# GuillaumeHolley/BloomFilterTrie

Hardware: AMD Instinct MI355X
Metric: M k-mers/sec queried (presenceNode) (higher is better)
Workload: dtype u64

## Files before the change

### bloomfiltertrie_amd/csrc/bft_kh.hip

```cpp
#include <hip/hip_runtime.h>

#include <algorithm>
#include <atomic>
#include <cstring>

#include "bft_dev.h"
#include "bft_image.h"
#include "bft_kh.h"
#include "bft_claims.h"
#include "bft_walk.h"
#include "bft_kernels_load.h"
#include "bft_kernels_seqwin.h"
#include "bft_kh_dev.h"
#include "bft_scan.h"
#include "bft_rows16.h"
#include "bft_sort.h"

#define BFT_KH_MIN_CLAIM 4u
#define BFT_KH_MAX_CLAIM 64u
typedef BftClaims<BFT_KH_MIN_CLAIM> KhClaims;
template <int W, int S>
__global__ __launch_bounds__(BFT_KH_BLOCK) void k_query_kh(BftImage im, const uint8_t* __restrict__ packed, uint64_t n, int B, uint64_t* __restrict__ bits64,
                                                          uint32_t* __restrict__ out32, BftClaimCtr ctr, uint32_t chunk) {
    const uint64_t end_aligned = ((uint64_t)packed + n * (uint64_t)B) & ~3ull;
    const uint64_t nblk = (n + BFT_KH_BLOCK - 1) / BFT_KH_BLOCK, nwords = (n + 63) / 64;
    constexpr uint32_t WPB = BFT_KH_BLOCK / 64;
    __shared__ uint32_t s_next[2];
    __shared__ uint64_t s_bits[BFT_KH_MAX_CLAIM * WPB];
    __shared__ uint4 s_lines[WPB][64 * BFT_KH_LDS_LINE];
    uint4* const wave_lines = s_lines[threadIdx.x >> 6];
    const uint4* const mine = wave_lines + (threadIdx.x & 63u) * BFT_KH_LDS_LINE;
    KhClaims cl(ctr, chunk, nblk, s_next);
    cl.first();
    while (cl.blk < nblk) {
        const uint64_t i = cl.blk * BFT_KH_BLOCK + threadIdx.x;
        const bool live = i < n;
        BftKhKey<W> key;
        key.home = 0;
        key.field = 0;
#pragma unroll
        for (int w = 0; w < W; w++) { key.body[w] = 0; key.bmask[w] = 0; }
        uint64_t t[W];
#pragma unroll
        for (int w = 0; w < W; w++) t[w] = 0;
        if (live) {
            uint64_t x[W];
            load_x<W>(packed, i, B, end_aligned, x);
            bft_tform_from_x<W>(x, im.k, t);
            bft_kh_key<W>(t, im.k, im.kh, key);
        }
        kh_fetch_quad(im, key.home, live, wave_lines);
        bool present = false;
        uint32_t val = 0xFFFFFFFFu;
        if (live) {
            int res = kh_lds_scan<W, S>(im, mine, key, 0u, &val);
            for (uint32_t d = 1; res < 0 && d <= im.kh.maxd; d++) {
                const uint64_t* line = im.kh_lines + (key.home + d) * BFT_KH_LINE_WORDS;
                uint64_t hd[2];
                bft_kh_load_header(line, hd);
                res = bft_kh_scan<W, S>(im, line, hd, key, d, &val);
            }
            if (res < 0 && im.kh_ovf_n) res = bft_kh_overflow_find<W>(im, t, &val) ? 1 : 0;
            present = res > 0;
        }
        const uint64_t mask = __ballot(present);
        if (out32 && i < n) out32[i] = present ? val : 0xFFFFFFFFu;
        if ((threadIdx.x & 63u) == 0) s_bits[(cl.blk - cl.start) * WPB + (threadIdx.x >> 6)] = mask;
        if (cl.last_of_round()) {
            __syncthreads();
            const uint64_t w0 = cl.start * WPB, w1 = min(nwords, cl.blk_end * WPB);
            if (w0 + threadIdx.x < w1) __builtin_nontemporal_store(s_bits[threadIdx.x], &bits64[w0 + threadIdx.x]);
        }
        cl.advance();
    }
    cl.done();
}

template <int W, int S>
__global__ __launch_bounds__(256) void k_color_rows_kh(BftImage im, const uint8_t* __restrict__ packed, uint64_t n, int B, uint64_t* __restrict__ bits64,
                                                       const uint8_t* __restrict__ bm, uint32_t stride, uint32_t rowbytes, uint32_t tile_rows, uint32_t div_m, uint32_t div_l,
                                                       uint8_t* __restrict__ out) {
    __shared__ uint4 s_lines[4][64 * BFT_KH_LDS_LINE];
    __shared__ uint32_t s_cs_all[4][BFT_KH_ROWS_TILE + 1];
    const uint64_t end_aligned = ((uint64_t)packed + n * (uint64_t)B) & ~3ull;
    const uint64_t ntiles = (n + tile_rows - 1) / tile_rows;
    const uint32_t lane = threadIdx.x & 63u, wave = threadIdx.x >> 6;
    uint4* const wave_lines = s_lines[wave];
    const uint4* const mine = wave_lines + lane * BFT_KH_LDS_LINE;
    uint32_t* const s_cs = s_cs_all[wave];
    for (uint64_t tile = (uint64_t)blockIdx.x * 4u + wave; tile < ntiles; tile += (uint64_t)gridDim.x * 4u) {
        const uint64_t q0 = tile * tile_rows;
        const uint32_t nt = (uint32_t)min((uint64_t)tile_rows, n - q0);
        __builtin_amdgcn_wave_barrier();
#pragma unroll 1
        for (uint32_t j0 = 0; j0 < nt; j0 += 64u) {
            const uint64_t i = q0 + j0 + lane;
            const bool live = i < n;
            BftKhKey<W> key;
            key.home = 0;
            key.field = 0;
#pragma unroll
            for (int w = 0; w < W; w++) { key.body[w] = 0; key.bmask[w] = 0; }
            uint64_t t[W];
#pragma unroll
            for (int w = 0; w < W; w++) t[w] = 0;
            if (live) {
                uint64_t x[W];
                load_x<W>(packed, i, B, end_aligned, x);
                bft_tform_from_x<W>(x, im.k, t);
                bft_kh_key<W>(t, im.k, im.kh, key);
            }
            kh_fetch_quad(im, key.home, live, wave_lines);
            bool present = false;
            uint32_t val = 0;
            if (live) {
                int res = kh_lds_scan<W, S>(im, mine, key, 0u, &val);
                for (uint32_t d = 1; res < 0 && d <= im.kh.maxd; d++) {
                    const uint64_t* line = im.kh_lines + (key.home + d) * BFT_KH_LINE_WORDS;
                    uint64_t hd[2];
                    bft_kh_load_header(line, hd);
                    res = bft_kh_scan<W, S>(im, line, hd, key, d, &val);
                }
                if (res < 0 && im.kh_ovf_n) res = bft_kh_overflow_find<W>(im, t, &val) ? 1 : 0;
                present = res > 0;
            }
            s_cs[j0 + lane] = present ? val * (stride >> 2) : CR16_ABSENT;
            const uint64_t mask = __ballot(present);
            if (lane == 0) bits64[(q0 + j0) >> 6] = mask;
        }
        if (lane == 0) s_cs[nt] = CR16_ABSENT;
        __builtin_amdgcn_fence(__ATOMIC_RELEASE, "wavefront");
        __builtin_amdgcn_wave_barrier();
        __builtin_amdgcn_fence(__ATOMIC_ACQUIRE, "wavefront");
        cr16_stream_tile(s_cs, nt, rowbytes, div_m, div_l, bm, out + q0 * rowbytes, lane);
    }
}

#ifndef BFT_KH_CT
#define BFT_KH_CT 4
#endif
#ifndef BFT_KH_LEN_T
#define BFT_KH_LEN_T uint16_t
#endif
template <int W, int S>
__global__ __launch_bounds__(BFT_KH_BLOCK) void k_colors_kh(BftImage im, const uint8_t* __restrict__ packed, uint64_t n, int B, uint64_t* __restrict__ bits64,
                                                           unsigned long long* __restrict__ offsets, uint32_t* __restrict__ ids, uint64_t ids_cap, unsigned long long* __restrict__ needed,
                                                           unsigned long long* __restrict__ scratch) {
    constexpr uint32_t WPB = BFT_KH_BLOCK / 64, CT = BFT_KH_CT;
    constexpr unsigned long long F_AGG = 1ull << 62, F_INC = 2ull << 62, VMASK = (1ull << 62) - 1ull;
    __shared__ uint4 s_lines[WPB][64 * BFT_KH_LDS_LINE];
    __shared__ uint64_t s_bits[CT * WPB];
    __shared__ uint32_t s_sum[CT * WPB];
    __shared__ BFT_KH_LEN_T s_len[CT * BFT_KH_BLOCK];
    __shared__ uint32_t s_src[CT * BFT_KH_BLOCK];
    __shared__ uint32_t s_tile;
    __shared__ unsigned long long s_prefix;
    const uint64_t end_aligned = ((uint64_t)packed + n * (uint64_t)B) & ~3ull;
    const uint32_t lane = threadIdx.x & 63u, wave = threadIdx.x >> 6;
    uint4* const wave_lines = s_lines[wave];
    const uint4* const mine = wave_lines + lane * BFT_KH_LDS_LINE;
    const uint64_t ntiles = (n + (uint64_t)CT * BFT_KH_BLOCK - 1) / ((uint64_t)CT * BFT_KH_BLOCK), nwords = (n + 63) / 64;
    unsigned long long* states = scratch + 1;
    for (;;) {
        if (threadIdx.x == 0) s_tile = (uint32_t)atomicAdd(scratch, 1ull);
        __syncthreads();
        const uint64_t tile = s_tile;
        if (tile >= ntiles) return;
#pragma unroll 1
        for (uint32_t c = 0; c < CT; c++) {
            const uint64_t i = (tile * CT + c) * BFT_KH_BLOCK + threadIdx.x;
            const bool live = i < n;
            BftKhKey<W> key;
            key.home = 0;
            key.field = 0;
#pragma unroll
            for (int w = 0; w < W; w++) { key.body[w] = 0; key.bmask[w] = 0; }
            uint64_t t[W];
#pragma unroll
            for (int w = 0; w < W; w++) t[w] = 0;
            if (live) {
                uint64_t x[W];
                load_x<W>(packed, i, B, end_aligned, x);
                bft_tform_from_x<W>(x, im.k, t);
                bft_kh_key<W>(t, im.k, im.kh, key);
            }
            kh_fetch_quad(im, key.home, live, wave_lines);
            bool present = false;
            uint32_t val = 0;
            if (live) {
                int res = kh_lds_scan<W, S>(im, mine, key, 0u, &val);
                for (uint32_t d = 1; res < 0 && d <= im.kh.maxd; d++) {
                    const uint64_t* line = im.kh_lines + (key.home + d) * BFT_KH_LINE_WORDS;
                    uint64_t hd[2];
                    bft_kh_load_header(line, hd);
                    res = bft_kh_scan<W, S>(im, line, hd, key, d, &val);
                }
                if (res < 0 && im.kh_ovf_n) res = bft_kh_overflow_find<W>(im, t, &val) ? 1 : 0;
                present = res > 0;
            }
            s_src[c * BFT_KH_BLOCK + threadIdx.x] = present ? val : 0xFFFFFFFFu;
            const uint64_t mask = __ballot(present);
            if (lane == 0) s_bits[c * WPB + wave] = mask;
        }
        {
            uint32_t cs[CT], o0[CT], o1[CT];
#pragma unroll
            for (uint32_t c = 0; c < CT; c++) cs[c] = s_src[c * BFT_KH_BLOCK + threadIdx.x];
#pragma unroll
            for (uint32_t c = 0; c < CT; c++) {
                o0[c] = 0; o1[c] = 0;
                if (cs[c] != 0xFFFFFFFFu) { o0[c] = im.cs_off[cs[c]]; o1[c] = im.cs_off[cs[c] + 1]; }
            }
#pragma unroll
            for (uint32_t c = 0; c < CT; c++) {
                const uint32_t len = o1[c] - o0[c];
                s_len[c * BFT_KH_BLOCK + threadIdx.x] = (BFT_KH_LEN_T)len;
                s_src[c * BFT_KH_BLOCK + threadIdx.x] = o0[c];
                uint32_t ws = len;
#pragma unroll
                for (int o = 32; o > 0; o >>= 1) ws += __shfl_down(ws, o);
                if (lane == 0) s_sum[c * WPB + wave] = ws;
            }
        }
        __syncthreads();
        {
            const uint64_t w0 = tile * CT * WPB;
            if (threadIdx.x < CT * WPB && w0 + threadIdx.x < nwords) __builtin_nontemporal_store(s_bits[threadIdx.x], &bits64[w0 + threadIdx.x]);
        }
        if (wave == 0) {
            unsigned long long total = lane < CT * WPB ? s_sum[lane] : 0u;
#pragma unroll
            for (int o = 32; o > 0; o >>= 1) total += __shfl_down(total, o);
            total = __shfl(total, 0);
            unsigned long long ex = 0;
            if (tile == 0) {
                if (lane == 0) __hip_atomic_store(&states[0], F_INC | (total & VMASK), __ATOMIC_RELAXED, __HIP_MEMORY_SCOPE_AGENT);
            } else {
                if (lane == 0) __hip_atomic_store(&states[tile], F_AGG | (total & VMASK), __ATOMIC_RELAXED, __HIP_MEMORY_SCOPE_AGENT);
                long long first = (long long)tile - 1;
                for (;;) {
                    const long long tt = first - (long long)lane;
                    unsigned long long st = F_INC;
                    if (tt >= 0) {
                        do { st = __hip_atomic_load(&states[tt], __ATOMIC_RELAXED, __HIP_MEMORY_SCOPE_AGENT); } while ((st >> 62) == 0ull && (__builtin_amdgcn_s_sleep(1), true));
                    }
                    const uint64_t incl = __ballot((st >> 62) == 2ull);
                    const int stop = incl ? __builtin_ctzll(incl) : 64;
                    unsigned long long x = ((int)lane <= stop && tt >= 0) ? (st & VMASK) : 0ull;
#pragma unroll
                    for (int o = 32; o > 0; o >>= 1) x += __shfl_down(x, o);
                    ex += __shfl(x, 0);
                    if (stop < 64) break;
                    first -= 64;
                }
                if (lane == 0) __hip_atomic_store(&states[tile], F_INC | ((ex + total) & VMASK), __ATOMIC_RELAXED, __HIP_MEMORY_SCOPE_AGENT);
            }
            if (lane == 0) {
                s_prefix = ex;
                if (tile == ntiles - 1) {
                    offsets[n] = ex + total;
                    if (needed) *needed = ex + total;
                }
            }
        }
        __syncthreads();
        unsigned long long run = s_prefix;
#pragma unroll 1
        for (uint32_t c = 0; c < CT; c++) {
            const uint32_t len = s_len[c * BFT_KH_BLOCK + threadIdx.x], src = s_src[c * BFT_KH_BLOCK + threadIdx.x];
            unsigned long long wbase = run;
#pragma unroll
            for (uint32_t w = 0; w < WPB; w++) {
                if (w < wave) wbase += s_sum[c * WPB + w];
                run += s_sum[c * WPB + w];
            }
            uint32_t inc = len;
#pragma unroll
            for (int o = 1; o < 64; o <<= 1) {
                const uint32_t y = __shfl_up(inc, o);
                if ((int)lane >= o) inc += y;
            }
            const uint32_t ar = inc - len, span = __shfl(inc, 63);
            const uint64_t i = (tile * CT + c) * BFT_KH_BLOCK + threadIdx.x;
            if (i < n) offsets[i] = wbase + ar;
            if (!ids) continue;
            for (uint32_t r0 = 0; r0 < span; r0 += 64) {
                const uint32_t r = r0 + lane;
                const bool in = r < span;
                const uint32_t rr = in ? r : span - 1;
                uint32_t lo = 0, hi = 63;
#pragma unroll
                for (int it = 0; it < 6; it++) {
                    const uint32_t mid = (lo + hi + 1) >> 1;
                    const uint32_t am = __shfl(ar, mid);
                    if (am <= rr) lo = mid; else hi = mid - 1;
                }
                const uint32_t as = __shfl(ar, lo);
                const uint32_t ss = __shfl(src, lo);
                if (in && wbase + r < ids_cap) ids[wbase + r] = bft_cs_id_at(im.cs_ids, im.cs_w, ss + (r - as));
            }
        }
        __syncthreads();
    }
}

template <int W, int S>
__device__ __forceinline__ int kh_count4(const BftImage& im, const uint64_t* t0, uint32_t b, int wild_word, int wild_shift, bool live, uint4* wave_lines) {
    BftKhKey<W> key;
    key.home = 0; key.field = 0;
#pragma unroll
    for (int w = 0; w < W; w++) { key.body[w] = 0; key.bmask[w] = 0; }
    if (live) bft_kh_key<W>(t0, im.k, im.kh, key);
    kh_fetch_quad(im, key.home, live, wave_lines);
    if (!live) return 0;
    BftKhFamily<W> fam;
    bft_kh_family<W>(im.kh, key, b, fam);
    int count = 0;
    int res = kh_lds_count<W, S>(im, wave_lines + (threadIdx.x & 63u) * BFT_KH_LDS_LINE, key, fam, 0u, &count);
    for (uint32_t d = 1; res < 0 && count < 4 && d <= im.kh.maxd; d++) res = bft_kh_count_line<W, S>(im, im.kh_lines + (key.home + d) * BFT_KH_LINE_WORDS, key, fam, d, &count);
    if (res < 0 && count < 4 && im.kh_ovf_n) {
        for (int v = 0; v < 4; v++) {
            uint64_t c[W];
            uint32_t val;
#pragma unroll
            for (int w = 0; w < W; w++) c[w] = t0[w] | (w == wild_word ? (uint64_t)v << wild_shift : 0ull);
            count += bft_kh_overflow_find<W>(im, c, &val) ? 1 : 0;
        }
    }
    return count;
}

#define BFT_KH_BR_MAX_CLAIM 16u
template <int W, int S>
__global__ __launch_bounds__(BFT_KH_BLOCK) void k_branching_kh(BftImage im, const uint8_t* __restrict__ packed, uint64_t n, int B, uint64_t* __restrict__ bits64,
                                                              uint8_t* __restrict__ counts, BftClaimCtr ctr, uint32_t chunk) {
    const uint64_t end_aligned = ((uint64_t)packed + n * (uint64_t)B) & ~3ull;
    const uint64_t nblk = (n + BFT_KH_BLOCK - 1) / BFT_KH_BLOCK, nwords = (n + 63) / 64;
    constexpr uint32_t WPB = BFT_KH_BLOCK / 64;
    const int k = im.k, L = im.L, rb = 2 * (k - 9 * L);
    __shared__ uint32_t s_next[2];
    __shared__ uint64_t s_bits[BFT_KH_BR_MAX_CLAIM * WPB];
    __shared__ uint4 s_lines[WPB][64 * BFT_KH_LDS_LINE];
    uint4* const wave_lines = s_lines[threadIdx.x >> 6];
    KhClaims cl(ctr, chunk, nblk, s_next);
    cl.first();
    while (cl.blk < nblk) {
        const uint64_t i = cl.blk * BFT_KH_BLOCK + threadIdx.x;
        const bool live = i < n;
        uint64_t x[W], y[W], t[W];
#pragma unroll
        for (int w = 0; w < W; w++) x[w] = 0;
        if (live) load_x<W>(packed, i, B, end_aligned, x);
#pragma unroll
        for (int w = 0; w < W; w++) y[w] = (x[w] >> 2) | (w + 1 < W ? x[w + 1] << 62 : 0ull);
        bft_tform_from_x<W>(y, k, t);
        const int vo = rb ? 0 : 2;
        const int cr = kh_count4<W, S>(im, t, (uint32_t)vo, W - 1, vo, live, wave_lines);
        int cl_ = 0;
        const bool left = live && (counts || cr < 2);
        if (__any(left)) {
#pragma unroll
            for (int w = W - 1; w >= 0; w--) y[w] = (x[w] << 2) | (w > 0 ? x[w - 1] >> 62 : 0ull);
            const int top = 2 * k - 64 * (W - 1);
            if (top < 64) y[W - 1] &= (1ull << top) - 1ull;
            bft_tform_from_x<W>(y, k, t);
            const int o = rb + 18 * (L - 1), ow = W - 1 - (o >> 6), osh = o & 63;
            cl_ = kh_count4<W, S>(im, t, im.kh.po < 32u ? im.kh.restb - 2u : (uint32_t)o, ow, osh, left, wave_lines);
        }
        const int branching = live && (cr > 1 || cl_ > 1);
        if (counts && live) counts[i] = (uint8_t)((cr << 4) | cl_);
        const uint64_t mask = __ballot(branching);
        if ((threadIdx.x & 63u) == 0) s_bits[(cl.blk - cl.start) * WPB + (threadIdx.x >> 6)] = mask;
        if (cl.last_of_round()) {
            __syncthreads();
            const uint64_t w0 = cl.start * WPB, w1 = min(nwords, cl.blk_end * WPB);
            if (w0 + threadIdx.x < w1) __builtin_nontemporal_store(s_bits[threadIdx.x], &bits64[w0 + threadIdx.x]);
        }
        cl.advance();
    }
    cl.done();
}

template <int W, int S>
__global__ __launch_bounds__(256) void k_seq_kh(BftImage im, const uint64_t* __restrict__ codes, const uint32_t* __restrict__ bad, const uint64_t* __restrict__ seq_off,
                                                const uint64_t* __restrict__ pos_off, const uint32_t* __restrict__ tile_seq, uint32_t n_seqs, int canonical,
                                                uint32_t* __restrict__ csout, BftClaimCtr ctr, uint32_t chunk) {
    const uint64_t P = pos_off[n_seqs];
    const uint64_t nblk = (P + 255) / 256;
    __shared__ uint32_t s_next[2];
    __shared__ uint4 s_lines[4][64 * BFT_KH_LDS_LINE];
    uint4* const wave_lines = s_lines[threadIdx.x >> 6];
    KhClaims cl(ctr, chunk, nblk, s_next);
    cl.first();
    for (; cl.blk < nblk; cl.advance()) {
        const uint64_t p = cl.blk * 256 + threadIdx.x;
        uint32_t cs = 0xFFFFFFFFu;
        uint64_t x[W], t[W];
        BftKhKey<W> key;
        key.home = 0; key.field = 0;
#pragma unroll
        for (int w = 0; w < W; w++) { key.body[w] = 0; key.bmask[w] = 0; }
        bool live = false;
        if (p < P) {
            uint32_t lo = tile_seq[p >> 6];
            while (lo + 1 < n_seqs && pos_off[lo + 1] <= p) lo++;
            if (seq_window<W>(codes, bad, seq_off[lo] + (p - pos_off[lo]), im.k, canonical, x)) {
                bft_tform_from_x<W>(x, im.k, t);
                bft_kh_key<W>(t, im.k, im.kh, key);
                live = true;
            }
        }
        kh_fetch_quad(im, key.home, live, wave_lines);
        if (live) {
            uint32_t val = 0;
            int res = kh_lds_scan<W, S>(im, wave_lines + (threadIdx.x & 63u) * BFT_KH_LDS_LINE, key, 0u, &val);
            for (uint32_t d = 1; res < 0 && d <= im.kh.maxd; d++) {
                const uint64_t* line = im.kh_lines + (key.home + d) * BFT_KH_LINE_WORDS;
                uint64_t hd[2];
                bft_kh_load_header(line, hd);
                res = bft_kh_scan<W, S>(im, line, hd, key, d, &val);
            }
            if (res < 0 && im.kh_ovf_n) res = bft_kh_overflow_find<W>(im, t, &val) ? 1 : 0;
            if (res > 0) cs = val;
        }
        if (p < P) csout[p] = cs;
    }
    cl.done();
}

template <int W>
struct __attribute__((packed, aligned(4))) KhRec {
    uint64_t t[W];
    uint32_t v;
};
template <int W>
struct KhSortIn {
    const uint64_t* tk;
    const uint32_t* vals;
    int k;
    BftKhGeo g;
    __device__ __forceinline__ uint32_t key(uint32_t i) const {
        uint64_t t[W];
        BftKhKey<W> kk;
        bft_load_row<W>(tk + (uint64_t)i * W, t);
        bft_kh_key<W>(t, k, g, kk);
        return (uint32_t)kk.home;
    }
    __device__ __forceinline__ KhRec<W> val(uint32_t i) const {
        KhRec<W> r;
        bft_load_row<W>(tk + (uint64_t)i * W, r.t);
        r.v = vals[i];
        return r;
    }
};
#define BFT_KH_SCAN_BIAS (1ull << 40)
struct KhScanIn {
    const uint32_t* key_s;
    uint32_t S;
    __device__ __forceinline__ uint64_t operator()(uint64_t s) const { return BFT_KH_SCAN_BIAS + (uint64_t)key_s[s] * S - s; }
};
template <int W>
__global__ __launch_bounds__(256) void k_kh_assemble(const uint32_t* __restrict__ key_s, const KhRec<W>* __restrict__ rec_s, const uint64_t* __restrict__ vscan, uint64_t n, int k,
                                                     BftKhGeo g, uint32_t* __restrict__ status, uint64_t* __restrict__ kh, uint64_t* __restrict__ ovf_k,
                                                     uint32_t* __restrict__ ovf_v) {
    __shared__ unsigned long long s_line[4][64][BFT_KH_LINE_WORDS];
    uint32_t dmax = 0;
    const uint64_t n_lines = g.nl + BFT_KH_TAIL_LINES;
    const uint32_t wave = threadIdx.x >> 6, lane = threadIdx.x & 63u;
    const uint64_t nblk = (n + 255) / 256;
    for (uint64_t blk = blockIdx.x; blk < nblk; blk += gridDim.x) {
        const uint64_t s = blk * 256 + threadIdx.x;
        const bool live = s < n;
        uint64_t p = 0, ln = ~0ull;
        bool first_of_line = false, last_of_line = false;
        if (live) {
            p = vscan[s] - BFT_KH_SCAN_BIAS + s;
            ln = p / g.S;
            first_of_line = s == 0 || (vscan[s - 1] - BFT_KH_SCAN_BIAS + (s - 1)) / g.S != ln;
            last_of_line = s + 1 == n || (vscan[s + 1] - BFT_KH_SCAN_BIAS + (s + 1)) / g.S != ln;
        }
        const uint64_t heads = __ballot(live && (first_of_line || lane == 0));
        const uint32_t rank = (uint32_t)__popcll(heads & ((2ull << lane) - 1ull)) - 1u;
        const uint64_t firsts = __ballot(live && first_of_line), lasts = __ballot(live && last_of_line);
        const uint64_t my_head_bit = live ? (1ull << (63 - __builtin_clzll((heads & ((2ull << lane) - 1ull)) | 1ull))) : 0ull;
        const uint64_t above = heads & ~((my_head_bit << 1) - 1ull);
        const uint32_t my_last_lane = above ? (uint32_t)__builtin_ctzll(above) - 1u : 63u;
        const bool whole = live && (firsts & my_head_bit) && my_last_lane < 64u && ((lasts >> my_last_lane) & 1ull);
#pragma unroll
        for (uint32_t q = 0; q < BFT_KH_LINE_WORDS; q++) s_line[wave][lane][q] = 0ull;
        __builtin_amdgcn_wave_barrier();
        uint64_t img[BFT_KH_LINE_WORDS];
#pragma unroll
        for (uint32_t q = 0; q < BFT_KH_LINE_WORDS; q++) img[q] = 0;
        if (live) {
            const uint64_t home = key_s[s], d = ln - home;
            const KhRec<W> r = rec_s[s];
            if (ln >= n_lines) atomicOr(&status[0], 1u);
            else if (d > g.maxd) {
                const uint32_t at = atomicAdd(&status[3], 1u);
                if (at >= BFT_KH_OVF_CAP) atomicOr(&status[0], 1u);
                else {
#pragma unroll
                    for (int w = 0; w < W; w++) ovf_k[(size_t)at * W + w] = r.t[w];
                    ovf_v[at] = r.v;
                }
                img[1] = 1ull << (64u - g.S + (uint32_t)(p % g.S));
            } else {
                dmax = max(dmax, (uint32_t)d);
                bft_kh_slot_image<W>(r.t, k, g, (uint32_t)(p % g.S), (uint32_t)d, r.v, img);
            }
            if (ln < n_lines) {
                if (whole) {
#pragma unroll
                    for (uint32_t q = 0; q < BFT_KH_LINE_WORDS; q++)
                        if (img[q]) atomicOr(&s_line[wave][rank][q], (unsigned long long)img[q]);
                } else {
                    unsigned long long* line = (unsigned long long*)(kh + ln * BFT_KH_LINE_WORDS);
#pragma unroll
                    for (uint32_t q = 0; q < BFT_KH_LINE_WORDS; q++)
                        if (img[q]) atomicOr(&line[q], (unsigned long long)img[q]);
                }
            }
        }
        __builtin_amdgcn_wave_barrier();
        if (whole && first_of_line && ln < n_lines) {
            ulonglong2* dst = reinterpret_cast<ulonglong2*>(kh + ln * BFT_KH_LINE_WORDS);
#pragma unroll
            for (int q = 0; q < 4; q++) dst[q] = make_ulonglong2(s_line[wave][rank][2 * q], s_line[wave][rank][2 * q + 1]);
        }
        __builtin_amdgcn_wave_barrier();
    }
    for (int o = 32; o > 0; o >>= 1) dmax = max(dmax, (uint32_t)__shfl_down(dmax, o));
    if ((threadIdx.x & 63u) == 0 && dmax) atomicMax(&status[2], dmax);
}

template <int W>
static int kh_sort_w(const uint64_t* d_tk, const uint32_t* d_vals, uint64_t n, int k, const BftKhGeo& g, BftKhScratch& sc, hipStream_t s) {
    DevBuf &key = sc.b[0], &rec = sc.b[1], &key_s = sc.b[2], &rec_s = sc.b[3], &tmp = sc.b[6];
    unsigned bits = 1;
    while (bits < 32 && (g.nl >> bits)) bits++;
    CK(key_s.alloc(n * 4));
    CK(rec_s.alloc(n * sizeof(KhRec<W>)));
    if (bft_rs::make_plan(0u, bits).P > 1) {
        CK(key.alloc(n * 4));
        CK(rec.alloc(n * sizeof(KhRec<W>)));
    }
    CK((bft_rs::sort<uint32_t, KhRec<W>, KhSortIn<W>, bft_rs::SHAPE_BACK>(KhSortIn<W>{d_tk, d_vals, k, g}, n, key_s.as<uint32_t>(), rec_s.as<KhRec<W>>(), key.as<uint32_t>(), rec.as<KhRec<W>>(), 0u, bits, s, tmp)));
    HIPCK(hipGetLastError());
    return 0;
}
template <int W>
static int kh_lay_w(uint64_t n, int k, const BftKhGeo& g, uint64_t* d_kh, uint64_t* d_ovf_k, uint32_t* d_ovf_v, uint32_t* d_status, BftKhScratch& sc,
                    hipStream_t s) {
    DevBuf &key_s = sc.b[2], &rec_s = sc.b[3], &vs = sc.b[5], &tmp = sc.b[6];
    CK(vs.alloc(n * 8));
    const dim3 b(256);
    HIPCK(hipMemsetAsync(d_status, 0, 16, s));
    HIPCK(hipMemsetAsync(d_kh, 0, (g.nl + BFT_KH_TAIL_LINES) * BFT_KH_LINE_WORDS * 8, s));
    CK((bft_scan::scan<uint64_t, KhScanIn, bft_scan::Max, true>(KhScanIn{key_s.as<uint32_t>(), g.S}, vs.as<uint64_t>(), n, 0ull, bft_scan::Max(), s, tmp)));
    hipLaunchKernelGGL(k_kh_assemble<W>, dim3((unsigned)std::min<uint64_t>((n + 255) / 256, 256ull * 32)), b, 0, s, key_s.as<uint32_t>(), rec_s.as<KhRec<W>>(), vs.as<uint64_t>(), n, k, g,
                       d_status, d_kh, d_ovf_k, d_ovf_v);
    HIPCK(hipGetLastError());
    return 0;
}

template <int W>
static int kh_test_sort_w(int shape, const uint32_t* keys, const void* recs, uint64_t n, unsigned b0, unsigned b1, uint32_t* ok, void* orec, hipStream_t s, uint32_t* h_dbase) {
    typedef bft_rs::PtrIn<uint32_t, KhRec<W>> In;
    const In in{keys, (const KhRec<W>*)recs};
    if (shape == bft_rs::SHAPE_BACK) return bft_rs::sort_test_run<uint32_t, KhRec<W>, In, bft_rs::SHAPE_BACK>(in, n, ok, (KhRec<W>*)orec, b0, b1, s, h_dbase);
    if (shape == bft_rs::SHAPE_BIG) return bft_rs::sort_test_run<uint32_t, KhRec<W>, In, bft_rs::SHAPE_BIG>(in, n, ok, (KhRec<W>*)orec, b0, b1, s, h_dbase);
    return bft_fail(BFT_GPU_E_ARG, "test sort: shape");
}
int bft_kh_test_sort(int W, int shape, const uint32_t* keys, const void* recs, uint64_t n, unsigned b0, unsigned b1, uint32_t* ok, void* orec, hipStream_t s, uint32_t* h_dbase) {
    switch (W) {
    case 1: return kh_test_sort_w<1>(shape, keys, recs, n, b0, b1, ok, orec, s, h_dbase);
    case 2: return kh_test_sort_w<2>(shape, keys, recs, n, b0, b1, ok, orec, s, h_dbase);
    case 3: return kh_test_sort_w<3>(shape, keys, recs, n, b0, b1, ok, orec, s, h_dbase);
    case 4: return kh_test_sort_w<4>(shape, keys, recs, n, b0, b1, ok, orec, s, h_dbase);
    default: return bft_fail(BFT_GPU_E_ARG, "test sort: W");
    }
}
template <int W>
static uint32_t kh_test_tile_w(int shape) {
    return shape == bft_rs::SHAPE_BACK ? bft_rs::tile_entries<uint32_t, KhRec<W>, bft_rs::SHAPE_BACK>()
         : shape == bft_rs::SHAPE_BIG  ? bft_rs::tile_entries<uint32_t, KhRec<W>, bft_rs::SHAPE_BIG>() : 0u;
}
uint32_t bft_kh_test_sort_tile(int W, int shape) {
    return W == 1 ? kh_test_tile_w<1>(shape) : W == 2 ? kh_test_tile_w<2>(shape) : W == 3 ? kh_test_tile_w<3>(shape) : W == 4 ? kh_test_tile_w<4>(shape) : 0u;
}

int bft_kh_sort(const uint64_t* d_tk, const uint32_t* d_vals, uint64_t n, int k, int W, const BftKhGeo& g, BftKhScratch& sc, hipStream_t s) {
    switch (W) {
    case 1: return kh_sort_w<1>(d_tk, d_vals, n, k, g, sc, s);
    case 2: return kh_sort_w<2>(d_tk, d_vals, n, k, g, sc, s);
    case 3: return kh_sort_w<3>(d_tk, d_vals, n, k, g, sc, s);
    default: return kh_sort_w<4>(d_tk, d_vals, n, k, g, sc, s);
    }
}
int bft_kh_lay(uint64_t n, int k, int W, const BftKhGeo& g, uint64_t* d_kh, uint64_t* d_ovf_k, uint32_t* d_ovf_v, uint32_t* d_status, BftKhScratch& sc, hipStream_t s) {
    switch (W) {
    case 1: return kh_lay_w<1>(n, k, g, d_kh, d_ovf_k, d_ovf_v, d_status, sc, s);
    case 2: return kh_lay_w<2>(n, k, g, d_kh, d_ovf_k, d_ovf_v, d_status, sc, s);
    case 3: return kh_lay_w<3>(n, k, g, d_kh, d_ovf_k, d_ovf_v, d_status, sc, s);
    default: return kh_lay_w<4>(n, k, g, d_kh, d_ovf_k, d_ovf_v, d_status, sc, s);
    }
}

template <int W>
__global__ __launch_bounds__(256) void k_kh_dump(BftImage im, uint64_t* __restrict__ keys, uint64_t stride, uint32_t* __restrict__ vals, unsigned long long* __restrict__ cnt) {
    __shared__ uint32_t s_cnt;
    __shared__ unsigned long long s_base;
    const uint64_t n_lines = im.kh.nl + BFT_KH_TAIL_LINES;
    const uint32_t S = im.kh.S;
    for (uint64_t l0 = (uint64_t)blockIdx.x * blockDim.x; l0 < n_lines; l0 += (uint64_t)gridDim.x * blockDim.x) {
        const uint64_t ln = l0 + threadIdx.x;
        if (threadIdx.x == 0) s_cnt = 0;
        __syncthreads();
        uint64_t hd[2] = {0, 0};
        uint32_t occ = 0;
        const uint64_t* line = im.kh_lines + ln * BFT_KH_LINE_WORDS;
        if (ln < n_lines) {
            bft_kh_load_header(line, hd);
            occ = (uint32_t)(hd[1] >> (64u - S));
        }
        {
            uint32_t real = 0;
            const uint64_t vmask = (1ull << im.kh.cb) - 1ull;
            for (uint32_t o2 = occ; o2;) {
                const uint32_t s = (uint32_t)__builtin_ctz(o2);
                o2 &= o2 - 1u;
                uint64_t body[W];
                bft_kh_load_body<W>(line, s, im.kh.wb, body);
                if (body[0] & vmask) real |= 1u << s;
            }
            occ = real;
        }
        const uint32_t mine = (uint32_t)__popc(occ);
        uint32_t my_off = mine ? atomicAdd(&s_cnt, mine) : 0u;
        __syncthreads();
        if (threadIdx.x == 0) s_base = s_cnt ? atomicAdd(cnt, (unsigned long long)s_cnt) : 0ull;
        __syncthreads();
        uint64_t j = s_base + my_off;
        while (occ) {
            const uint32_t s = (uint32_t)__builtin_ctz(occ);
            occ &= occ - 1u;
            uint64_t t[W];
            uint32_t v;
            bft_kh_slot_decode<W>(im, line, hd, ln, s, t, &v);
#pragma unroll
            for (int i = 0; i < W; i++) keys[(uint64_t)i * stride + j] = t[i];
            vals[j] = v;
            j++;
        }
        __syncthreads();
    }
    if (blockIdx.x == 0) {
        __syncthreads();
        if (threadIdx.x == 0) s_base = im.kh_ovf_n ? atomicAdd(cnt, (unsigned long long)im.kh_ovf_n) : 0ull;
        __syncthreads();
        for (uint32_t e = threadIdx.x; e < im.kh_ovf_n; e += blockDim.x) {
#pragma unroll
            for (int i = 0; i < W; i++) keys[(uint64_t)i * stride + s_base + e] = im.kh_ovf[(size_t)e * W + i];
            vals[s_base + e] = im.kh_ovf_val[e];
        }
    }
}

int bft_kh_dump(const BftImage& im, uint64_t* d_keys, uint64_t stride, uint32_t* d_vals, unsigned long long* d_cnt, hipStream_t s) {
    const dim3 grid(256 * 8), block(256);
    switch (im.W) {
    case 1: hipLaunchKernelGGL(k_kh_dump<1>, grid, block, 0, s, im, d_keys, stride, d_vals, d_cnt); break;
    case 2: hipLaunchKernelGGL(k_kh_dump<2>, grid, block, 0, s, im, d_keys, stride, d_vals, d_cnt); break;
    case 3: hipLaunchKernelGGL(k_kh_dump<3>, grid, block, 0, s, im, d_keys, stride, d_vals, d_cnt); break;
    default: hipLaunchKernelGGL(k_kh_dump<4>, grid, block, 0, s, im, d_keys, stride, d_vals, d_cnt); break;
    }
    HIPCK(hipGetLastError());
    return 0;
}

bool bft_kh_has_kernels(int W, uint32_t S) {
    switch (W) {
    case 1: return S >= 4 && S <= 10;
    case 2: return S >= 3 && S <= 10;
    case 3: return S >= 2 && S <= 4;
    default: return S >= 1 && S <= 2;
    }
}

static dim3 kh_round_grid(uint64_t n, uint32_t chunk, int mult, bool claimed) {
    const uint64_t nblk = (n + BFT_KH_BLOCK - 1) / BFT_KH_BLOCK, rounds = (nblk + chunk - 1) / chunk;
    const uint64_t resident = 256ull * 8 * (uint64_t)std::max(1, mult) * (claimed ? 1ull : 4ull);
    return dim3((unsigned)std::max<uint64_t>(1, std::min<uint64_t>(rounds, resident)));
}

int bft_kh_query(const BftImage& im, int grid_mult, const uint8_t* d_kmers, uint64_t n, int rec, uint64_t* d_bits64, uint32_t* d_out32, BftClaimCtr d_ctr, uint32_t chunk,
                 hipStream_t s) {
    const dim3 block(BFT_KH_BLOCK);
    chunk = std::max(1u, std::min(chunk, BFT_KH_MAX_CLAIM));
    const dim3 grid = kh_round_grid(n, chunk, grid_mult, d_ctr.p != nullptr);
    KH_DISPATCH(im.W, (int)im.kh.S, hipLaunchKernelGGL((k_query_kh<KW, KS>), grid, block, 0, s, im, d_kmers, n, rec, d_bits64, d_out32, d_ctr, chunk));
    HIPCK(hipGetLastError());
    return 0;
}

size_t bft_kh_colors_scratch_bytes(uint64_t n) { return ((n + (uint64_t)BFT_KH_CT * BFT_KH_BLOCK - 1) / ((uint64_t)BFT_KH_CT * BFT_KH_BLOCK) + 1) * 8; }
int bft_kh_colors(const BftImage& im, const uint8_t* d_kmers, uint64_t n, int rec, uint64_t* d_bits64, uint64_t* d_offsets, uint32_t* d_ids, uint64_t ids_cap, uint64_t* d_needed,
                  void* d_scratch, hipStream_t s) {
    const uint64_t ntiles = (n + (uint64_t)BFT_KH_CT * BFT_KH_BLOCK - 1) / ((uint64_t)BFT_KH_CT * BFT_KH_BLOCK);
    CK(bft_zero_async(d_scratch, (ntiles + 1) * 8, s));
    const dim3 grid((unsigned)std::max<uint64_t>(1, std::min<uint64_t>(ntiles, 256ull * 8))), block(BFT_KH_BLOCK);
    KH_DISPATCH(im.W, (int)im.kh.S,
                hipLaunchKernelGGL((k_colors_kh<KW, KS>), grid, block, 0, s, im, d_kmers, n, rec, d_bits64, (unsigned long long*)d_offsets, d_ids, ids_cap, (unsigned long long*)d_needed,
                                   (unsigned long long*)d_scratch));
    HIPCK(hipGetLastError());
    return 0;
}

template <int W, int S>
static void kh_color_rows_launch(const BftImage& im, const uint8_t* d_kmers, uint64_t n, int rec, uint64_t* d_bits64, const uint8_t* bm, uint32_t stride, uint32_t rowbytes,
                                 uint32_t tile_rows, uint32_t div_m, uint32_t div_l, uint8_t* d_out, int device, hipStream_t s) {
    static std::atomic<int> resident_dev[64];
    std::atomic<int>& res = resident_dev[device & 63];
    int r = res.load(std::memory_order_relaxed);
    if (!r) {
        int per_cu = 0, cus = 0;
        if (hipOccupancyMaxActiveBlocksPerMultiprocessor(&per_cu, k_color_rows_kh<W, S>, 256, 0) != hipSuccess || per_cu < 1) { per_cu = 4; (void)hipGetLastError(); }
        if (hipDeviceGetAttribute(&cus, hipDeviceAttributeMultiprocessorCount, device) != hipSuccess || cus < 1) { cus = 256; (void)hipGetLastError(); }
        r = per_cu * cus;
        res.store(r, std::memory_order_relaxed);
    }
    const uint64_t tiles = (n + tile_rows - 1) / tile_rows;
    const dim3 grid((unsigned)std::max<uint64_t>(1, std::min<uint64_t>((tiles + 3) / 4, (uint64_t)r)));
    hipLaunchKernelGGL((k_color_rows_kh<W, S>), grid, dim3(256), 0, s, im, d_kmers, n, rec, d_bits64, bm, stride, rowbytes, tile_rows, div_m, div_l, d_out);
}

int bft_kh_color_rows(const BftImage& im, const uint8_t* d_kmers, uint64_t n, int rec, uint64_t* d_bits64, const uint8_t* bm, uint32_t stride, uint32_t rowbytes, uint8_t* d_out,
                      int device, hipStream_t s) {
    const BftColorRowsPlan plan = bft_color_rows_plan(rowbytes, BFT_ROWS_FORM_KH);
    KH_DISPATCH(im.W, (int)im.kh.S, (kh_color_rows_launch<KW, KS>(im, d_kmers, n, rec, d_bits64, bm, stride, rowbytes, plan.tile_rows, plan.div_m, plan.div_l, d_out, device, s)));
    HIPCK(hipGetLastError());
    return 0;
}

int bft_kh_branching(const BftImage& im, const uint8_t* d_kmers, uint64_t n, int B, uint64_t* d_bits64, uint8_t* d_counts, BftClaimCtr d_ctr, uint32_t chunk, hipStream_t s) {
    const dim3 block(BFT_KH_BLOCK);
    chunk = std::max(1u, std::min(chunk, BFT_KH_BR_MAX_CLAIM));
    const dim3 grid = kh_round_grid(n, chunk, 1, d_ctr.p != nullptr);
    KH_DISPATCH(im.W, (int)im.kh.S, hipLaunchKernelGGL((k_branching_kh<KW, KS>), grid, block, 0, s, im, d_kmers, n, B, d_bits64, d_counts, d_ctr, chunk));
    HIPCK(hipGetLastError());
    return 0;
}

int bft_kh_seq(const BftImage& im, const uint64_t* d_codes, const uint32_t* d_bad, const uint64_t* d_seq_off, const uint64_t* d_pos_off, const uint32_t* d_tile_seq,
               uint32_t n_seqs, int canonical, uint32_t* d_csout, BftClaimCtr d_ctr, uint32_t chunk, hipStream_t s) {
    const dim3 grid(256 * 8), block(256);
    chunk = std::max(1u, std::min(chunk, BFT_KH_MAX_CLAIM));
    KH_DISPATCH(im.W, (int)im.kh.S,
                hipLaunchKernelGGL((k_seq_kh<KW, KS>), grid, block, 0, s, im, d_codes, d_bad, d_seq_off, d_pos_off, d_tile_seq, n_seqs, canonical, d_csout, d_ctr, chunk));
    HIPCK(hipGetLastError());
    return 0;
}
```

Baseline: 52810.

## Replace per-element max-scan with bucketed per-64-line carry scan in KH assembly

The kh hash-table layout now processes buckets of 64 home lines per wavefront. A bucket kernel binary-searches each bucket's start and computes a per-bucket max term, and a small scan over buckets yields the carry. Assembly then reconstructs slot positions with ballot-based in-wave histograms instead of reading a full n-sized 64-bit scan array. The radix sort skips the low 6 bits, since the bucket kernels order within a bucket themselves. This removes the n-element scan and its memory traffic at the cost of more intricate wave-level logic. It only affects the build path, so the query metric probably does not move.

```diff
diff --git a/bloomfiltertrie_amd/csrc/bft_kh.hip b/bloomfiltertrie_amd/csrc/bft_kh.hip
--- a/bloomfiltertrie_amd/csrc/bft_kh.hip
+++ b/bloomfiltertrie_amd/csrc/bft_kh.hip
@@ -453,68 +453,151 @@
         return r;
     }
 };
-#define BFT_KH_SCAN_BIAS (1ull << 40)
-struct KhScanIn {
-    const uint32_t* key_s;
-    uint32_t S;
-    __device__ __forceinline__ uint64_t operator()(uint64_t s) const { return BFT_KH_SCAN_BIAS + (uint64_t)key_s[s] * S - s; }
+#define BFT_KH_BUCKET_BITS 6u
+
+struct KhChunk {
+    uint64_t bj[BFT_KH_BUCKET_BITS], on;
+    __device__ __forceinline__ KhChunk(uint32_t l, bool has) {
+        on = __ballot(has);
+#pragma unroll
+        for (uint32_t q = 0; q < BFT_KH_BUCKET_BITS; q++) bj[q] = __ballot(has && ((l >> q) & 1u));
+    }
+    __device__ __forceinline__ uint64_t lanes_of(uint32_t h) const {
+        uint64_t m = on;
+#pragma unroll
+        for (uint32_t q = 0; q < BFT_KH_BUCKET_BITS; q++) m &= ((h >> q) & 1u) ? bj[q] : ~bj[q];
+        return m;
+    }
 };
+__device__ __forceinline__ uint32_t kh_bucket_hist(const uint32_t* __restrict__ key_s, uint32_t s0, uint32_t s1, uint32_t lane) {
+    uint32_t c = 0;
+    for (uint32_t i = s0; i < s1; i += 64u) {
+        const bool has = i + lane < s1;
+        const uint32_t l = has ? key_s[i + lane] & 63u : 0u;
+        const KhChunk ch(l, has);
+        c += (uint32_t)__popcll(ch.lanes_of(lane));
+    }
+    return c;
+}
+__device__ __forceinline__ void kh_bucket_terms(uint32_t c, uint32_t s0, uint64_t line0, uint32_t S, uint32_t lane, uint32_t& before, uint64_t& term) {
+    uint32_t inc = c;
+#pragma unroll
+    for (int o = 1; o < 64; o <<= 1) {
+        const uint32_t y = __shfl_up(inc, o);
+        if ((int)lane >= o) inc += y;
+    }
+    before = inc - c;
+    const uint64_t hs = (line0 + lane) * S, F = (uint64_t)s0 + before;
+    term = c && hs > F ? hs - F : 0ull;
+}
+__global__ __launch_bounds__(256) void k_kh_buckets(const uint32_t* __restrict__ key_s, uint32_t n, uint32_t nb, uint32_t S, uint32_t* __restrict__ bstart,
+                                                    uint64_t* __restrict__ bmax) {
+    const uint32_t wave = threadIdx.x >> 6, lane = threadIdx.x & 63u;
+    for (uint64_t b64 = (uint64_t)blockIdx.x * 4u + wave; b64 < nb; b64 += (uint64_t)gridDim.x * 4u) {
+        const uint32_t b = (uint32_t)b64;
+        uint32_t lo = 0, hi = n;
+        while (hi - lo > 64u) {
+            const uint32_t step = (hi - lo + 63u) / 64u;
+            const uint64_t at = (uint64_t)lo + (uint64_t)(lane + 1u) * step - 1u;
+            const bool below = at < hi && (key_s[at] >> BFT_KH_BUCKET_BITS) < b;
+            const uint32_t cnt = (uint32_t)__popcll(__ballot(below));
+            lo += cnt * step;
+            hi = min(hi, lo + step - 1u);
+        }
+        {
+            const bool below = lo + lane < hi && (key_s[lo + lane] >> BFT_KH_BUCKET_BITS) < b;
+            lo += (uint32_t)__popcll(__ballot(below));
+        }
+        uint32_t c = 0;
+        for (uint32_t i = lo; i < n; i += 64u) {
+            const uint32_t key = i + lane < n ? key_s[i + lane] : 0xFFFFFFFFu;
+            const bool has = i + lane < n && (key >> BFT_KH_BUCKET_BITS) == b;
+            const KhChunk ch(key & 63u, has);
+            c += (uint32_t)__popcll(ch.lanes_of(lane));
+            if (ch.on != ~0ull) break;
+        }
+        uint32_t before;
+        uint64_t term;
+        kh_bucket_terms(c, lo, (uint64_t)b << BFT_KH_BUCKET_BITS, S, lane, before, term);
+#pragma unroll
+        for (int o = 32; o > 0; o >>= 1) {
+            const uint64_t y = bft_scan::shfl_t(term, (int)((lane + o) & 63u));
+            term = term > y ? term : y;
+        }
+        if (lane == 0) {
+            bstart[b] = lo;
+            bmax[b] = term;
+            if (b + 1u == nb) bstart[nb] = n;
+        }
+    }
+}
 template <int W>
-__global__ __launch_bounds__(256) void k_kh_assemble(const uint32_t* __restrict__ key_s, const KhRec<W>* __restrict__ rec_s, const uint64_t* __restrict__ vscan, uint64_t n, int k,
-                                                     BftKhGeo g, uint32_t* __restrict__ status, uint64_t* __restrict__ kh, uint64_t* __restrict__ ovf_k,
-                                                     uint32_t* __restrict__ ovf_v) {
+__global__ __launch_bounds__(256) void k_kh_assemble(const uint32_t* __restrict__ key_s, const KhRec<W>* __restrict__ rec_s, const uint32_t* __restrict__ bstart,
+                                                     const uint64_t* __restrict__ carry, uint32_t nb, int k, BftKhGeo g, uint32_t* __restrict__ status, uint64_t* __restrict__ kh,
+                                                     uint64_t* __restrict__ ovf_k, uint32_t* __restrict__ ovf_v) {
     __shared__ unsigned long long s_line[4][64][BFT_KH_LINE_WORDS];
     uint32_t dmax = 0;
     const uint64_t n_lines = g.nl + BFT_KH_TAIL_LINES;
     const uint32_t wave = threadIdx.x >> 6, lane = threadIdx.x & 63u;
-    const uint64_t nblk = (n + 255) / 256;
-    for (uint64_t blk = blockIdx.x; blk < nblk; blk += gridDim.x) {
-        const uint64_t s = blk * 256 + threadIdx.x;
-        const bool live = s < n;
-        uint64_t p = 0, ln = ~0ull;
-        bool first_of_line = false, last_of_line = false;
-        if (live) {
-            p = vscan[s] - BFT_KH_SCAN_BIAS + s;
-            ln = p / g.S;
-            first_of_line = s == 0 || (vscan[s - 1] - BFT_KH_SCAN_BIAS + (s - 1)) / g.S != ln;
-            last_of_line = s + 1 == n || (vscan[s + 1] - BFT_KH_SCAN_BIAS + (s + 1)) / g.S != ln;
-        }
-        const uint64_t heads = __ballot(live && (first_of_line || lane == 0));
-        const uint32_t rank = (uint32_t)__popcll(heads & ((2ull << lane) - 1ull)) - 1u;
-        const uint64_t firsts = __ballot(live && first_of_line), lasts = __ballot(live && last_of_line);
-        const uint64_t my_head_bit = live ? (1ull << (63 - __builtin_clzll((heads & ((2ull << lane) - 1ull)) | 1ull))) : 0ull;
-        const uint64_t above = heads & ~((my_head_bit << 1) - 1ull);
-        const uint32_t my_last_lane = above ? (uint32_t)__builtin_ctzll(above) - 1u : 63u;
-        const bool whole = live && (firsts & my_head_bit) && my_last_lane < 64u && ((lasts >> my_last_lane) & 1ull);
+    const uint64_t lt_mask = (1ull << lane) - 1ull;
+    for (uint64_t b64 = (uint64_t)blockIdx.x * 4u + wave; b64 < nb; b64 += (uint64_t)gridDim.x * 4u) {
+        const uint32_t s0 = bstart[b64], s1 = bstart[b64 + 1];
+        if (s0 == s1) continue;
+        const uint64_t cy = carry[b64], line0 = b64 << BFT_KH_BUCKET_BITS;
 #pragma unroll
         for (uint32_t q = 0; q < BFT_KH_LINE_WORDS; q++) s_line[wave][lane][q] = 0ull;
+        const uint32_t c = kh_bucket_hist(key_s, s0, s1, lane);
+        uint32_t before;
+        uint64_t m;
+        kh_bucket_terms(c, s0, line0, g.S, lane, before, m);
+#pragma unroll
+        for (int o = 1; o < 64; o <<= 1) {
+            const uint64_t y = bft_scan::shfl_up_t(m, o);
+            if ((int)lane >= o && y > m) m = y;
+        }
+        const uint64_t base = (uint64_t)s0 + before + (m > cy ? m : cy);
+        const uint64_t own_lo = s0 ? max(line0, ((uint64_t)s0 - 1u + cy) / g.S + 1u) : line0, own_hi = min(line0 + 64u, g.nl);
+        __builtin_amdgcn_fence(__ATOMIC_RELEASE, "wavefront");
         __builtin_amdgcn_wave_barrier();
-        uint64_t img[BFT_KH_LINE_WORDS];
-#pragma unroll
-        for (uint32_t q = 0; q < BFT_KH_LINE_WORDS; q++) img[q] = 0;
-        if (live) {
-            const uint64_t home = key_s[s], d = ln - home;
-            const KhRec<W> r = rec_s[s];
-            if (ln >= n_lines) atomicOr(&status[0], 1u);
-            else if (d > g.maxd) {
-                const uint32_t at = atomicAdd(&status[3], 1u);
-                if (at >= BFT_KH_OVF_CAP) atomicOr(&status[0], 1u);
-                else {
-#pragma unroll
-                    for (int w = 0; w < W; w++) ovf_k[(size_t)at * W + w] = r.t[w];
-                    ovf_v[at] = r.v;
+        __builtin_amdgcn_fence(__ATOMIC_ACQUIRE, "wavefront");
+        uint32_t seen = 0;
+        for (uint32_t i = s0; i < s1; i += 64u) {
+            const uint32_t s = i + lane;
+            const bool has = s < s1;
+            const uint32_t home = has ? key_s[s] : (uint32_t)line0;
+            const uint32_t l = home & 63u;
+            const KhChunk ch(l, has);
+            const uint32_t r = __shfl(seen, (int)l) + (uint32_t)__popcll(ch.lanes_of(l) & lt_mask);
+            seen += (uint32_t)__popcll(ch.lanes_of(lane));
+            const uint64_t p = bft_scan::shfl_t(base, (int)l) + r;
+            if (has) {
+                const KhRec<W> rec = rec_s[s];
+                const uint64_t rel = p - line0 * g.S;
+                const uint64_t lr = (rel >> 32) ? rel / g.S : (uint64_t)((uint32_t)rel / g.S);
+                const uint32_t slot = (uint32_t)(rel - lr * g.S);
+                const uint64_t ln = line0 + lr, d = ln - home;
+                uint64_t img[BFT_KH_LINE_WORDS];
+#pragma unroll
+                for (uint32_t q = 0; q < BFT_KH_LINE_WORDS; q++) img[q] = 0;
+                if (ln >= n_lines) atomicOr(&status[0], 1u);
+                else if (d > g.maxd) {
+                    const uint32_t at = atomicAdd(&status[3], 1u);
+                    if (at >= BFT_KH_OVF_CAP) atomicOr(&status[0], 1u);
+                    else {
+#pragma unroll
+                        for (int w = 0; w < W; w++) ovf_k[(size_t)at * W + w] = rec.t[w];
+                        ovf_v[at] = rec.v;
+                    }
+                    img[1] = 1ull << (64u - g.S + slot);
+                } else {
+                    dmax = max(dmax, (uint32_t)d);
+                    bft_kh_slot_image<W>(rec.t, k, g, slot, (uint32_t)d, rec.v, img);
                 }
-                img[1] = 1ull << (64u - g.S + (uint32_t)(p % g.S));
-            } else {
-                dmax = max(dmax, (uint32_t)d);
-                bft_kh_slot_image<W>(r.t, k, g, (uint32_t)(p % g.S), (uint32_t)d, r.v, img);
-            }
-            if (ln < n_lines) {
-                if (whole) {
+                if (ln >= own_lo && ln < own_hi) {
 #pragma unroll
                     for (uint32_t q = 0; q < BFT_KH_LINE_WORDS; q++)
-                        if (img[q]) atomicOr(&s_line[wave][rank][q], (unsigned long long)img[q]);
-                } else {
+                        if (img[q]) atomicOr(&s_line[wave][lr][q], (unsigned long long)img[q]);
+                } else if (ln < n_lines) {
                     unsigned long long* line = (unsigned long long*)(kh + ln * BFT_KH_LINE_WORDS);
 #pragma unroll
                     for (uint32_t q = 0; q < BFT_KH_LINE_WORDS; q++)
@@ -522,16 +605,22 @@
                 }
             }
         }
+        __builtin_amdgcn_fence(__ATOMIC_RELEASE, "wavefront");
         __builtin_amdgcn_wave_barrier();
-        if (whole && first_of_line && ln < n_lines) {
-            ulonglong2* dst = reinterpret_cast<ulonglong2*>(kh + ln * BFT_KH_LINE_WORDS);
-#pragma unroll
-            for (int q = 0; q < 4; q++) dst[q] = make_ulonglong2(s_line[wave][rank][2 * q], s_line[wave][rank][2 * q + 1]);
-        }
+        __builtin_amdgcn_fence(__ATOMIC_ACQUIRE, "wavefront");
+#pragma unroll
+        for (uint32_t q = 0; q < 4; q++) {
+            const uint32_t e = q * 64u + lane, wl = e >> 2, part = e & 3u;
+            const uint64_t ln = line0 + wl;
+            if (ln >= own_lo && ln < own_hi)
+                *reinterpret_cast<ulonglong2*>(kh + ln * BFT_KH_LINE_WORDS + 2u * part) = make_ulonglong2(s_line[wave][wl][2u * part], s_line[wave][wl][2u * part + 1u]);
+        }
+        __builtin_amdgcn_fence(__ATOMIC_RELEASE, "wavefront");
         __builtin_amdgcn_wave_barrier();
+        __builtin_amdgcn_fence(__ATOMIC_ACQUIRE, "wavefront");
     }
     for (int o = 32; o > 0; o >>= 1) dmax = max(dmax, (uint32_t)__shfl_down(dmax, o));
-    if ((threadIdx.x & 63u) == 0 && dmax) atomicMax(&status[2], dmax);
+    if (lane == 0 && dmax > __hip_atomic_load(&status[2], __ATOMIC_RELAXED, __HIP_MEMORY_SCOPE_AGENT)) atomicMax(&status[2], dmax);
 }
 
 template <int W>
@@ -539,27 +628,34 @@
     DevBuf &key = sc.b[0], &rec = sc.b[1], &key_s = sc.b[2], &rec_s = sc.b[3], &tmp = sc.b[6];
     unsigned bits = 1;
     while (bits < 32 && (g.nl >> bits)) bits++;
+    bits = std::max(bits, BFT_KH_BUCKET_BITS);
     CK(key_s.alloc(n * 4));
     CK(rec_s.alloc(n * sizeof(KhRec<W>)));
-    if (bft_rs::make_plan(0u, bits).P > 1) {
+    if (bft_rs::make_plan(BFT_KH_BUCKET_BITS, bits).P > 1) {
         CK(key.alloc(n * 4));
         CK(rec.alloc(n * sizeof(KhRec<W>)));
     }
-    CK((bft_rs::sort<uint32_t, KhRec<W>, KhSortIn<W>, bft_rs::SHAPE_BACK>(KhSortIn<W>{d_tk, d_vals, k, g}, n, key_s.as<uint32_t>(), rec_s.as<KhRec<W>>(), key.as<uint32_t>(), rec.as<KhRec<W>>(), 0u, bits, s, tmp)));
+    CK((bft_rs::sort<uint32_t, KhRec<W>, KhSortIn<W>, bft_rs::SHAPE_BACK>(KhSortIn<W>{d_tk, d_vals, k, g}, n, key_s.as<uint32_t>(), rec_s.as<KhRec<W>>(), key.as<uint32_t>(), rec.as<KhRec<W>>(),
+                                                                          BFT_KH_BUCKET_BITS, bits, s, tmp)));
     HIPCK(hipGetLastError());
     return 0;
 }
 template <int W>
 static int kh_lay_w(uint64_t n, int k, const BftKhGeo& g, uint64_t* d_kh, uint64_t* d_ovf_k, uint32_t* d_ovf_v, uint32_t* d_status, BftKhScratch& sc,
                     hipStream_t s) {
-    DevBuf &key_s = sc.b[2], &rec_s = sc.b[3], &vs = sc.b[5], &tmp = sc.b[6];
-    CK(vs.alloc(n * 8));
-    const dim3 b(256);
+    DevBuf &key_s = sc.b[2], &rec_s = sc.b[3], &bk = sc.b[5], &tmp = sc.b[6];
+    const uint64_t nb = (g.nl + 63) >> BFT_KH_BUCKET_BITS;
+    CK(bk.alloc(nb * 16 + (nb + 1) * 4));
+    uint64_t* const d_carry = bk.as<uint64_t>();
+    uint64_t* const d_bmax = d_carry + nb;
+    uint32_t* const d_bstart = reinterpret_cast<uint32_t*>(d_bmax + nb);
+    const dim3 b(256), grid((unsigned)std::min<uint64_t>((nb + 3) / 4, 256ull * 32));
     HIPCK(hipMemsetAsync(d_status, 0, 16, s));
     HIPCK(hipMemsetAsync(d_kh, 0, (g.nl + BFT_KH_TAIL_LINES) * BFT_KH_LINE_WORDS * 8, s));
-    CK((bft_scan::scan<uint64_t, KhScanIn, bft_scan::Max, true>(KhScanIn{key_s.as<uint32_t>(), g.S}, vs.as<uint64_t>(), n, 0ull, bft_scan::Max(), s, tmp)));
-    hipLaunchKernelGGL(k_kh_assemble<W>, dim3((unsigned)std::min<uint64_t>((n + 255) / 256, 256ull * 32)), b, 0, s, key_s.as<uint32_t>(), rec_s.as<KhRec<W>>(), vs.as<uint64_t>(), n, k, g,
-                       d_status, d_kh, d_ovf_k, d_ovf_v);
+    hipLaunchKernelGGL(k_kh_buckets, grid, b, 0, s, key_s.as<uint32_t>(), (uint32_t)n, (uint32_t)nb, g.S, d_bstart, d_bmax);
+    HIPCK(hipGetLastError());
+    CK((bft_scan::scan<uint64_t, bft_scan::PtrIn<uint64_t>, bft_scan::Max, false>(bft_scan::PtrIn<uint64_t>{d_bmax}, d_carry, nb, 0ull, bft_scan::Max(), s, tmp)));
+    hipLaunchKernelGGL(k_kh_assemble<W>, grid, b, 0, s, key_s.as<uint32_t>(), rec_s.as<KhRec<W>>(), d_bstart, d_carry, (uint32_t)nb, k, g, d_status, d_kh, d_ovf_k, d_ovf_v);
     HIPCK(hipGetLastError());
     return 0;
 }
```

Result: no change. 52860 (median of 2 runs) (+0.1%).
